# SketchyScene/SketchySceneColorization

Hardware: AMD Instinct MI355X
Metric: train images/sec (192x192, gen+disc fwd+bwd) (higher is better)
Workload: dtype fp32 (bf16x6 split on the bf16 MFMA, fp32 accumulate; filter gradients and few-channel layers on the exact-fp32 MFMA)

## Files before the change

include/sketchycolor_hip.h:

```cpp
#ifndef SKETCHYCOLOR_HIP_H
#define SKETCHYCOLOR_HIP_H

#include <stdint.h>

#ifdef __cplusplus
extern "C" {
#endif

#define SSC_ACT_NONE 0
#define SSC_ACT_RELU 1
#define SSC_ACT_LRELU 2
#define SSC_ACT_TANH 3
#define SSC_ACT_PRELU 5
#define SSC_ACT_MIU 4

typedef struct ssc_gview {
    const float* s0;
    const float* s1;
    const float* ab0;
    const float* ab1;
    int32_t C0, C1;
    int32_t H, W;
    int32_t act;
    int32_t act1;
// ... 46 lines not shown
    void* dst;
    int32_t taps, c0, c1, orient;
    int64_t first_thread;
} ssc_split_job;
int ssc_filter_split_geom(int taps, int c0, int c1, int orient, int* kc, int* nbp, int64_t* bytes, int64_t* threads);
int ssc_filter_split(const float* w, int taps, int c0, int c1, int orient, void* dst, void* stream);
int ssc_bf16_prepare(void);
int ssc_filter_split_batch(const ssc_split_job* jobs_dev, int njobs, int64_t total_threads, void* stream);

int ssc_sk_configure(int timeout_ms, int test_withhold);

typedef struct ssc_wgrad_desc {
    ssc_gview g;
    ssc_gview d;
    float* out;
    int32_t NB, PH, PW;
    int32_t TH, TW, in_stride, ioff_y, ioff_x;
    int32_t Cg_real;
    int32_t Nn;
    int32_t ldc;
    int32_t accumulate;
    int32_t exact;
    int32_t _pad;
} ssc_wgrad_desc;

int ssc_version(void);
int ssc_build_hash(char* buf, int len);
int ssc_device_info(int* cu_count, int* wave_size, char* arch, int arch_len);

int ssc_conv_forward(const ssc_conv_desc* d, float* ws, int64_t ws_bytes, void* stream);
int ssc_conv_wgrad(const ssc_wgrad_desc* d, float* ws, int64_t ws_bytes, void* stream);
int ssc_conv_wgrad128_supported(const ssc_wgrad_desc* d);
int ssc_conv_wgrad128(const ssc_wgrad_desc* d, float* ws, int64_t ws_bytes, void* stream);
int ssc_conv_wgn16_supported(const ssc_wgrad_desc* d);
int ssc_conv_forward_bn(const ssc_conv_desc* d, float* ws, int64_t ws_bytes, const float* scale, const float* offset,
                        float eps, float* ab, float* stats, void* stream);
int ssc_head1_forward_supported(const ssc_conv_desc* d);
int ssc_head1_forward(const ssc_conv_desc* d, float* ws, int64_t ws_bytes, void* stream);
int ssc_head1_dgrad_supported(const ssc_conv_desc* d);
int ssc_head1_dgrad(const ssc_conv_desc* d, void* stream);
int ssc_head1_wgrad_supported(const ssc_wgrad_desc* d);
int ssc_head1_wgrad(const ssc_wgrad_desc* d, float* ws, int64_t ws_bytes, void* stream);
int ssc_head1_dgrad_bn_backward(const ssc_conv_desc* d, const float* x, const float* ab, const float* stats, int act,
                                const float* rowb, float rowb_scale, float* dx, float* dscale, float* doffset, float* ws,
                                int64_t ws_bytes, void* stream);
int ssc_bn_bwd_finalize(const float* partial, int nblk, int C, int64_t M, float* coef, float* dscale, float* doffset,
                        void* stream);
int ssc_conv_narrow_supported(const ssc_conv_desc* d);
int ssc_conv_narrow_forward(const ssc_conv_desc* d, void* stream);
int ssc_conv_pw1x1_supported(const ssc_conv_desc* d);
int ssc_conv_c3x3_supported(const ssc_conv_desc* d);
int ssc_conv_s2n16_supported(const ssc_conv_desc* d);
int ssc_conv_tr4n16_supported(const ssc_conv_desc* d);
int ssc_conv_fewchan7_supported(const ssc_conv_desc* d);
int ssc_conv_tr4_tiny_supported(const ssc_conv_desc* d);
int ssc_conv_fewchan_supported(const ssc_conv_desc* d);
int ssc_conv_forward_kernel_name(const ssc_conv_desc* d, char* buf, int len);
int ssc_conv_wgrad_kernel_name(const ssc_wgrad_desc* d, char* buf, int len);
int ssc_conv_forward_plan(const ssc_conv_desc* d, int64_t ws_bytes, int* out5);
int ssc_conv_wgrad_plan(const ssc_wgrad_desc* d, int64_t ws_bytes, int* out4);
int ssc_conv_wgrad128_plan(const ssc_wgrad_desc* d, int64_t ws_bytes, int* out7);
int ssc_conv_bf_plan(const ssc_conv_desc* d, int64_t ws_bytes, int* out10);

int ssc_nchw_to_nhwc(const float* src, float* dst, int N, int C, int HW, int ldc, int coff, void* stream);
int ssc_nhwc_to_nchw(const float* src, float* dst, int N, int C, int HW, int ldc, int coff, void* stream);
int ssc_sketch_preprocess_u8(const uint8_t* src, int N, int H, int W, int thicken, float* dst, void* stream);
int ssc_image_postprocess_u8(const float* src, int ldc, int coff, int64_t M, uint8_t* dst, void* stream);
int ssc_bg_stage_u8(const uint8_t* fg, const uint8_t* bg, const int32_t* labels, int64_t M, float* inputs, float* targets,
                    float* xd_real, float* count, void* workspace, int64_t workspace_bytes, void* stream);
int ssc_bg_stage_cached_u8(const uint8_t* fg_cache, int64_t S_fg, const uint8_t* bg_cache, int64_t S_bg, const uint8_t* seg_cache,
                           int64_t S_seg, const int32_t* slot, const uint8_t* recolor, int64_t N, int64_t P, float* inputs,
                           float* targets, float* xd_real, int32_t* labels, float* count, void* workspace,
                           int64_t workspace_bytes, void* stream);
int ssc_bg_finish_u8(const float* img, int ldc, const uint8_t* fg, const uint8_t* mask, int64_t M, uint8_t* out,
                     void* stream);
int ssc_image_metrics_u8(const uint8_t* a, const uint8_t* b, const uint8_t* mask, int N, int H, int W, const double* win11,
                         double* out, void* ws, int64_t ws_bytes, void* stream);
int ssc_image_metrics_f32(const float* a, int lda, int coff_a, const float* b, int ldb, int coff_b, int b_planar, int N, int H,
                          int W, const double* win11, double* out, void* ws, int64_t ws_bytes, void* stream);
int ssc_image_metrics_bg_f32(const float* img, int ldc, const uint8_t* fg, const uint8_t* target, const uint8_t* mask, int N, int H,
                             int W, const double* win11, double* out, void* ws, int64_t ws_bytes, void* stream);
int ssc_seg_confusion(const float* logits, int ld, int K, const int32_t* labels, int64_t N, int64_t P, int64_t* out, void* ws,
                      int64_t ws_bytes, void* stream);
int ssc_bg_scene_crop_u8(const uint8_t* prev, const uint8_t* inner, int64_t M, uint8_t* fg_out, void* stream);
int ssc_bg_scene_compose_u8(const float* img, int ldc, const uint8_t* fg, const uint8_t* inner, const uint8_t* grass,
                            const uint8_t* sketch, int H, int W, uint8_t* out, uint8_t* fg_marked, int overlay_only,
                            void* stream);
int ssc_bg_sky_gradient_u8(const uint8_t* color, const uint8_t* inner, int H, int W, int search_from, int search_height,
                           uint8_t* out, int32_t* status, void* workspace, int64_t workspace_bytes, void* stream);
int ssc_fg_scene_mask_u8(const uint8_t* small_mask, int bh, int bw, uint8_t* out, void* stream);
int ssc_road_parallel_u8(const uint8_t* sketch, int S, int parallel_width, int32_t* out, void* stream);
int ssc_fg_scene_paste_u8(uint8_t* result, const uint8_t* inner, int H, int W, const uint8_t* inst, int y1, int x1, int bh, int bw,
                          int value, void* stream);
int ssc_resample_u8(const uint8_t* src, int H, int W, int C, int chan, const int32_t* bnd_h, const int32_t* k_h, int ks_h,
                    int new_w, const int32_t* bnd_v, const int32_t* k_v, int ks_v, int new_h, uint8_t* tmp, uint8_t* dst,
                    int OH, int OW, int OC, int top, int left, int fill, void* stream);
int ssc_decode_paired_u8(const uint8_t* img, const uint8_t* sk, const float* sk_f32, int N, int R, int size,
                         const float* noise, float* img_out, float* sk_out, float* mnmx, void* stream);
int ssc_decode_minmax_u8(const uint8_t* img, int N, int R, int size, float* mnmx, void* stream);
int ssc_decode_paired_cached_u8(const uint8_t* img_cache, const uint8_t* sk_cache, const float* skf_cache,
                                const float* mnmx_cache, int64_t S, const int32_t* idx, int N, int R, int size,
                                const float* noise, float* img_out, float* sk_out, void* stream);
int ssc_distance_map_u8(const uint8_t* sk, int N, int R, float* out, int32_t* ws, int64_t ws_bytes, void* stream);
uint32_t ssc_crc32c(const uint8_t* data, int64_t n);
int ssc_fill(float* dst, float value, int64_t n, void* stream);
int ssc_timestamp(uint64_t* dst, void* stream);
// ... 206 lines not shown
```

sketchyscenecolorization_amd/build.py:

```python
import os
import subprocess
import sys

HERE = os.path.dirname(os.path.abspath(__file__))
ROOT = os.path.dirname(HERE)
CSRC = os.path.join(HERE, 'csrc')
LIB_DIR = os.path.join(HERE, 'lib')
LIB_PATH = os.path.join(LIB_DIR, 'libsketchycolor_hip.so')
EXTRA_FLAGS = {'igemm.hip': ['-Xclang', '-target-feature', '-Xclang', '-load-store-opt']} if os.environ.get('SSC_NO_LSOPT') == '1' else {}
NO_PACKED_FP32 = {'narrow.hip': []}
VGPR_FORM = ['-mllvm', '-amdgpu-mfma-vgpr-form=1']
LAST_BUILD = None
SOURCES = ['igemm.hip', 'igemm_bf16.hip', 'wgrad128.hip', 'wgrad128_bf16.hip', 'wgn16.hip', 'narrow.hip', 'head1.hip', 'fewchan.hip', 'fewchan7.hip', 'pw1x1.hip', 'c3x3.hip', 's2n16.hip', 'tr4tiny.hip', 'tr4n16.hip', 'elementwise.hip', 'text_lstm.hip', 'losses_optim.hip', 'mru_ops.hip', 'bg_io.hip', 'bg_scene.hip', 'fg_scene.hip', 'metrics.hip', 'matching.hip', 'match_eval.hip', 'match_train.hip', 'match_val.hip', 'match_backbone_train.hip', 'match_attn.hip', 'match_segnet.hip']


def _hipcc():
    for c in (os.environ.get('HIPCC'), '/opt/rocm/bin/hipcc', 'hipcc'):
        if c and (os.path.isabs(c) and os.path.exists(c) or not os.path.isabs(c)):
            return c
    return 'hipcc'


HASH_MARKER = b'SSC_CSRC_HASH='


def tree_hash(csrc=None, header=None):
    import hashlib
    csrc = csrc or CSRC
    header = header or os.path.join(ROOT, 'include', 'sketchycolor_hip.h')
    h = hashlib.sha256()
    for fp in [os.path.join(csrc, f) for f in sorted(os.listdir(csrc))] + [header]:
        if fp.endswith(('.hip', '.h')):
            with open(fp, 'rb') as fh:
                h.update(os.path.basename(fp).encode() + b'\0' + fh.read())
    return h.hexdigest()[:16]


def library_hash(path=None):
    path = path or LIB_PATH
    if not os.path.exists(path):
        return None
    with open(path, 'rb') as fh:
        blob = fh.read()
    i = blob.find(HASH_MARKER)
    if i < 0:
        return None
    return blob[i + len(HASH_MARKER):i + len(HASH_MARKER) + 16].decode('ascii', 'replace')


def is_stale():
    return library_hash() != tree_hash()


def build_library(force=False, verbose=True):
    global LAST_BUILD
    if not force and not is_stale():
        LAST_BUILD = 'reused'
        return LIB_PATH
    LAST_BUILD = 'rebuilt'
    os.makedirs(LIB_DIR, exist_ok=True)
    th = tree_hash()
    import hashlib
    objs = []
    procs = []
    hdrs = b''
    for hp in sorted(os.path.join(CSRC, f) for f in os.listdir(CSRC) if f.endswith('.h')) + [os.path.join(ROOT, 'include', 'sketchycolor_hip.h')]:
# ... 36 lines not shown
```

sketchyscenecolorization_amd/csrc/igemm.hip:

```cpp
#include <hip/hip_runtime.h>
#include <stdint.h>
#include <stdio.h>
#include <stdlib.h>
#include "sketchycolor_hip.h"
#include "igemm_util.h"
#include "igemm_epilogue.h"
#include "host_util.h"

extern "C" int ssc_conv_wgrad128_supported(const ssc_wgrad_desc* dp);
extern "C" int ssc_conv_wgrad128(const ssc_wgrad_desc* dp, float* ws, int64_t ws_bytes, void* stream);
int ssc_conv_wgrad128_bf_selected(const ssc_wgrad_desc* dp);
extern "C" int ssc_conv_wgn16_supported(const ssc_wgrad_desc* dp);
int ssc_conv_wgn16(const ssc_wgrad_desc* dp, float* ws, int64_t ws_bytes, void* stream);
int ssc_conv_wgn16_fits(const ssc_wgrad_desc* dp, int64_t ws_bytes);
int ssc_conv_narrow_forward_ws(const ssc_conv_desc* dp, float* ws, int64_t ws_bytes, void* stream, int* csplit_out);
int ssc_conv_fewchan_forward(const ssc_conv_desc* dp, int num_cu, void* stream);
extern "C" int ssc_conv_pw1x1_supported(const ssc_conv_desc* dp);
int ssc_conv_pw1x1_walkers(const ssc_conv_desc* dp);
int ssc_conv_pw1x1_forward(const ssc_conv_desc* dp, float* stat, void* stream);
extern "C" int ssc_conv_tr4n16_supported(const ssc_conv_desc* dp);
int ssc_conv_tr4n16_rows(const ssc_conv_desc* dp);
int ssc_conv_tr4n16_forward(const ssc_conv_desc* dp, float* stat, void* stream);
extern "C" int ssc_conv_fewchan7_supported(const ssc_conv_desc* dp);
int ssc_conv_fewchan7_walkers(const ssc_conv_desc* dp);
int ssc_conv_fewchan7_forward(const ssc_conv_desc* dp, float* stat, void* stream);
extern "C" int ssc_conv_tr4_tiny_supported(const ssc_conv_desc* dp);
int ssc_conv_tr4_tiny_blocks(const ssc_conv_desc* dp);
int ssc_conv_tr4_tiny_forward(const ssc_conv_desc* dp, float* stat, void* stream);
extern "C" int ssc_conv_s2n16_supported(const ssc_conv_desc* dp);
int ssc_conv_s2n16_walkers(const ssc_conv_desc* dp);
int ssc_conv_s2n16_forward(const ssc_conv_desc* dp, float* stat, void* stream);
extern "C" int ssc_conv_c3x3_supported(const ssc_conv_desc* dp);
int ssc_conv_c3x3_walkers(const ssc_conv_desc* dp);
int ssc_conv_c3x3_forward(const ssc_conv_desc* dp, float* stat, void* stream);

bool ssc_bf_hk_enabled();
int ssc_launch_conv_bf(int cfg, bool plain, const ssc_conv_desc& d, int splitk, float* ws, hipStream_t st, long ts_full, int ts_s,
                       int64_t ws_bytes, int xcd);
int ssc_conv_bf_form(int cfg, bool plain, const ssc_conv_desc& d, int splitk, bool have_ws, long ts_full, int ts_s, int64_t ws_bytes,
                     int xcd, int* out10);
int ssc_sk_configure_bf(const unsigned* cfg4);

#define BK 32
__device__ unsigned g_sk_cfg[4] = {2000000000u, 0u, 0u, 0u};
#ifndef SSC_BDMA
#define SSC_BDMA 1
#endif
#ifndef SSC_ADMA
#define SSC_ADMA 0
#endif
#ifndef SSC_UT_SGB
#define SSC_UT_SGB 1
#endif

template <int WM, int WN, int SM, int SN, int BMODE, bool VECB>
__global__ __launch_bounds__(256) void conv_fwd_kernel(const ssc_conv_desc d, const Magics mg,
                                                        float* __restrict__ slab_base, long slab_stride,
                                                        int splitk) {
    constexpr int BM = WM * SM * 32;
    constexpr int BN = WN * SN * 32;
    constexpr int A_LD = BK + 1;
    constexpr int A_SZ = BM * A_LD;
    constexpr int B_LD = (BMODE == 0) ? BN : (BK + 1);
    constexpr int B_SZ = (BMODE == 0) ? BK * BN : BN * (BK + 1);
    constexpr int A_ROWS = BM / 32;
    constexpr int B_SLOTS = BN / 32;
    constexpr int B_RP = 1024 / BN;
    static_assert(WM * WN == 4, "4 waves per workgroup");

    extern __shared__ __attribute__((aligned(16))) float smem[];
    float* As = smem;
    float* Bs = smem + 2 * A_SZ;
    long* rowpix = reinterpret_cast<long*>(smem + 2 * A_SZ + 2 * B_SZ);

    const int tid = threadIdx.x;
// ... 1379 lines not shown
        const char* e = getenv("SSC_ARITH");
        off = (e != nullptr && (e[0] == 'f' || e[0] == 'F')) ? 1 : 0;
    }
    const bool km = d.x.C1 == 0 && (d.x.C0 & 3) == 0 && d.x.C0 > BK && (d.x.C0 % BK) != 0 && d.k_real >= 1 && d.k_real <= d.x.C0 &&
                    d.ws_kc == 2 * ((d.x.C0 + BK - 1) / BK) && (long)d.NB * d.x.H * d.x.W * d.x.C0 < 0x1fffffffL &&
                    (long)d.KH * d.KW * d.wC0 * d.wC1 < 0x1fffffffL;
    return !off && d.wsplit != nullptr && d.ws_kc > 0 && d.ws_nbp > 0 && (fwd_is_ut(d) || km) && (d.n_off & 31) == 0 && d.Nstore > 32 &&
           d.TH * d.TW <= 32;
}

static Plan plan_fwd(const ssc_conv_desc& d, int64_t ws_bytes, bool have_ws) {
    const long M = (long)d.NB * d.PH * d.PW;
    const int C = d.x.C0 + d.x.C1;
    long nkt = ((long)d.TH * d.TW * C + BK - 1) / BK;
    if (fwd_is_ut(d) || fwd_is_utg(d))
        nkt = (long)d.TH * d.TW * ((d.x.C0 + BK - 1) / BK + (d.x.C1 + BK - 1) / BK);
    else if (d.bmode == 0 && fwd_is_rowtap(d))
        nkt = d.TH;
    const bool allowed[5] = {d.Nstore > 64, d.Nstore > 64, d.Nstore > 32, d.Nstore <= 32, d.Nstore > 32};
    const bool can_ts = d.sk_flags != nullptr && tail_split_mode() != 0 &&
                        (fwd_is_ut(d) || fwd_is_utg(d) || (d.bmode == 0 && fwd_is_rowtap(d)));
    if (fwd_is_bf(d)) {
        const bool allowed_bf[5] = {d.Nstore > 64, d.Nstore > 64, true, false, true};
        TileCfg cfgs[5];
        for (int i = 0; i < 5; ++i) cfgs[i] = BF_CFGS[i];
        if (ssc_bf_hk_enabled()) {
            const long t128 = ((M + 127) / 128) * ((d.Nstore + 127) / 128) * d.nphase;
            if ((double)t128 < plan_const("SSC_PLAN_BF_HK_MIN", 0.5) * 2.0 * num_cu()) {
                return plan_launch(cfgs, 5, allowed_bf, M, d.Nstore, d.nphase, nkt, (long)d.NB * d.OH * d.OW * d.ldc, ws_bytes,
                                   have_ws, can_ts, plan_const("SSC_PLAN_BF_SCALE", 0.45));
            }
            cfgs[0].res = 2;
            cfgs[0].penalty = plan_const("SSC_PLAN_BF_HK", 0.78);
            if (!fwd_is_ut(d)) cfgs[0].penalty *= (double)((d.x.C0 + 15) / 16) / (double)(2 * ((d.x.C0 + 31) / 32));
        }
        return plan_launch(cfgs, 5, allowed_bf, M, d.Nstore, d.nphase, nkt, (long)d.NB * d.OH * d.OW * d.ldc, ws_bytes,
                           have_ws, can_ts, plan_const("SSC_PLAN_BF_SCALE", 0.45));
    }
    return plan_launch(FWD_CFGS, 5, allowed, M, d.Nstore, d.nphase, nkt, (long)d.NB * d.OH * d.OW * d.ldc, ws_bytes,
                       have_ws, can_ts);
}

static void copy_name(const char* src, char* dst, int len) {
    int i = 0;
    for (; i < len - 1 && src[i]; ++i) dst[i] = src[i];
    if (len > 0) dst[i] = 0;
}

extern "C" int ssc_conv_forward_kernel_name(const ssc_conv_desc* dp, char* buf, int len) {
    if (ssc_head1_forward_supported(dp) || ssc_head1_dgrad_supported(dp)) {
        copy_name(ssc_head1_dgrad_supported(dp) ? "head1_dgrad" : "head1_fwd", buf, len);
        return 0;
    }
    if (ssc_conv_narrow_supported(dp)) {
        copy_name(dp->nphase == 4 ? "narrow_fwd<transposed>" : "narrow_fwd<conv>", buf, len);
        return 0;
    }
    if (ssc_conv_fewchan_supported(dp)) {
        copy_name(dp->x.C0 == 8 ? "conv_fewchan<8>" : "conv_fewchan<4>", buf, len);
        return 0;
    }
    if (ssc_conv_pw1x1_supported(dp)) {
        copy_name("conv_pw1x1", buf, len);
        return 0;
    }
    if (ssc_conv_c3x3_supported(dp)) {
        copy_name(dp->bmode ? "conv_c3x3<NK>" : "conv_c3x3<KN>", buf, len);
        return 0;
    }
    if (ssc_conv_s2n16_supported(dp)) {
        copy_name("conv_s2n16", buf, len);
        return 0;
    }
    if (ssc_conv_tr4_tiny_supported(dp)) {
        copy_name("deconv_tr4_tiny", buf, len);
        return 0;
    }
    if (ssc_conv_fewchan7_supported(dp)) {
        copy_name("conv_fewchan7", buf, len);
        return 0;
    }
    if (ssc_conv_tr4n16_supported(dp)) {
        copy_name("deconv_tr4n16", buf, len);
        return 0;
    }
    static const char* names[2][5] = {
        {"conv_fwd<128x128,KN>", "conv_fwd<64x128,KN>", "conv_fwd<128x64,KN>", "conv_fwd<128x32,KN>", "conv_fwd<64x64,KN>"},
        {"conv_fwd<128x128,NK>", "conv_fwd<64x128,NK>", "conv_fwd<128x64,NK>", "conv_fwd<128x32,NK>", "conv_fwd<64x64,NK>"}};
    const Plan p = plan_fwd(*dp, (int64_t)1 << 40, true);
    if (fwd_is_bf(*dp)) {
        static const char* bfn[5] = {"conv_bf16x6<128x128>", "conv_bf16x6<64x128>", "conv_bf16x6<128x64>", "conv_bf16x6<128x32>",
                                     "conv_bf16x6<64x64>"};
        copy_name(bfn[p.cfg < 0 ? 0 : p.cfg], buf, len);
        return 0;
    }
    copy_name(names[dp->bmode ? 1 : 0][p.cfg < 0 ? 0 : p.cfg], buf, len);
    return 0;
}

extern "C" int ssc_bn_stats(const float* x, int64_t M, int C, int ldx, const float* scale, const float* offset, float eps,
                            float* ab, float* stats, float* ws, int64_t ws_bytes, void* stream);
extern "C" int ssc_bn_finalize(const float* partial, int nblk, int C, int64_t M, const float* scale, const float* offset,
                               float eps, float* ab, float* stats, void* stream);

extern "C" int ssc_conv_forward_bn(const ssc_conv_desc* dp, float* ws, int64_t ws_bytes, const float* scale,
                                   const float* offset, float eps, float* ab, float* stats, void* stream) {
// ... 192 lines not shown
        const char* e = ssc_dev_getenv("SSC_FUSE_BNBWD");
        off = (e != nullptr && e[0] == '0') ? 1 : 0;
    }
    const int C1 = d.Nstore - C0;
    if (!off && ws != nullptr && s0 != nullptr && s1 != nullptr && s0->x && s1->x && s0->ab && s1->ab && s0->stats && s1->stats &&
        s0->partial && s1->partial && C0 > 0 && C1 > 0 && (C0 % 128) == 0 && (C1 & 3) == 0 &&
        !ssc_conv_narrow_supported(dp) && !ssc_conv_fewchan_supported(dp) && d.epi == 0 && !d.accumulate &&
        d.bias == nullptr && d.Nstore == d.ldc && d.Nn == d.Nstore && ((s0->ldx | s1->ldx) & 3) == 0 &&
        ((reinterpret_cast<unsigned long>(d.out) | reinterpret_cast<unsigned long>(s0->x) |
          reinterpret_cast<unsigned long>(s1->x)) & 15) == 0 &&
        (fwd_is_ut(d) || fwd_is_utg(d))) {
        const Plan p = plan_fwd(d, ws_bytes, true);
        if (p.cfg >= 0 && p.splitk == 1 && FWD_CFGS[p.cfg].BN <= 128) {
            const long mt = (M + FWD_CFGS[p.cfg].BM - 1) / FWD_CFGS[p.cfg].BM;
            if ((int64_t)mt * d.nphase * 2 * C0 * 4 <= s0->partial_bytes && (int64_t)mt * d.nphase * 2 * C1 * 4 <= s1->partial_bytes) {
                d.stat_partial = s0->partial;
                d.sb_x = s0->x; d.sb_ldx = s0->ldx; d.sb_ab = s0->ab; d.sb_stats = s0->stats; d.sb_act = s0->act;
                d.stat_partial2 = s1->partial; d.sb2_col0 = C0;
                d.sb2_x = s1->x; d.sb2_ldx = s1->ldx; d.sb2_ab = s1->ab; d.sb2_stats = s1->stats; d.sb2_act = s1->act;
                *nrows = (int)(mt * d.nphase);
            }
        }
    }
    return ssc_conv_forward(&d, ws, ws_bytes, stream);
}

extern "C" int ssc_sk_configure(int timeout_ms, int test_withhold) {
    const unsigned long long ticks = (unsigned long long)(timeout_ms > 0 ? timeout_ms : 20000) * 100000ull;
    const unsigned cfg[4] = {(unsigned)(ticks & 0xffffffffu), (unsigned)(ticks >> 32), test_withhold ? 1u : 0u, 0u};
    const int rc = ssc_sk_configure_bf(cfg);
    if (rc != 0) return rc;
    return (int)hipMemcpyToSymbol(HIP_SYMBOL(g_sk_cfg), cfg, sizeof(cfg), 0, hipMemcpyHostToDevice);
}

extern "C" int ssc_conv_forward_plan(const ssc_conv_desc* dp, int64_t ws_bytes, int* out5) {
    if (ssc_conv_narrow_supported(dp) || ssc_conv_fewchan_supported(dp)) {
        out5[0] = -1; out5[1] = 1; out5[2] = 0; out5[3] = 1; out5[4] = 0;
        return 0;
    }
    const Plan p = plan_fwd(*dp, ws_bytes, true);
    out5[0] = p.cfg; out5[1] = p.splitk; out5[2] = (int)p.ts_full; out5[3] = p.ts_s; out5[4] = (int)(p.cost / 1000.0);
    return 0;
}

static int fwd_desc_error(const ssc_conv_desc& d) {
    if ((d.x.C0 & 3) || (d.x.C1 & 3) || d.Nstore < d.Nn || d.Nstore > d.ldc) return -1;
    if (d.nphase != 1 && d.nphase != 4) return -2;
    if (d.nphase == 4 && (d.TH != 2 || d.TW != 2 || d.KH != 4 || d.KW != 4 || d.kstep != -2 || d.out_stride != 2 ||
                          d.in_stride != 1))
        return -3;
    return 0;
}
enum { FWD_TILED = 0, FWD_HEAD1, FWD_HEAD1_DGRAD, FWD_NARROW, FWD_FEWCHAN, FWD_PW1X1, FWD_C3X3, FWD_S2N16, FWD_TR4_TINY, FWD_FEWCHAN7,
       FWD_TR4N16 };
static int fwd_early_kernel(const ssc_conv_desc* dp, bool have_ws, int64_t ws_bytes) {
    const ssc_conv_desc& d = *dp;
    if (have_ws && ssc_head1_forward_supported(dp) && (int64_t)d.NB * d.x.H * d.x.W * 16 * 4 <= ws_bytes) return FWD_HEAD1;
    if (ssc_head1_dgrad_supported(dp)) return FWD_HEAD1_DGRAD;
    if (ssc_conv_narrow_supported(dp)) return FWD_NARROW;
    if (ssc_conv_fewchan_supported(dp)) return FWD_FEWCHAN;
    if (ssc_conv_pw1x1_supported(dp)) return FWD_PW1X1;
    if (ssc_conv_c3x3_supported(dp)) return FWD_C3X3;
    if (ssc_conv_s2n16_supported(dp)) return FWD_S2N16;
    if (ssc_conv_tr4_tiny_supported(dp)) return FWD_TR4_TINY;
    if (ssc_conv_fewchan7_supported(dp)) return FWD_FEWCHAN7;
    if (ssc_conv_tr4n16_supported(dp)) return FWD_TR4N16;
    return FWD_TILED;
}
static bool fwd_bf_plain(const ssc_conv_desc& d) {
    const bool plain0 = d.x.ab0 == nullptr && d.x.act == SSC_ACT_NONE;
    const bool plain1 = d.x.C1 == 0 || (d.x.ab1 == nullptr && (d.x.act1 >= 0 ? d.x.act1 : d.x.act) == SSC_ACT_NONE);
    return plain0 && plain1;
}

extern "C" int ssc_conv_bf_plan(const ssc_conv_desc* dp, int64_t ws_bytes, int* out10) {
    const ssc_conv_desc& d = *dp;
    const bool have_ws = ws_bytes > 0;
    const int err = fwd_desc_error(d);
    if (err != 0) return err;
    if (fwd_early_kernel(dp, have_ws, ws_bytes) != FWD_TILED || !fwd_is_bf(d)) return -10;
    const Plan p = plan_fwd(d, ws_bytes, have_ws);
    if (p.cfg < 0) return -4;
    return ssc_conv_bf_form(p.cfg, fwd_bf_plain(d), d, p.splitk, have_ws, p.ts_full, p.ts_s, ws_bytes, xcd_order(), out10);
}

extern "C" int ssc_conv_forward(const ssc_conv_desc* dp, float* ws, int64_t ws_bytes, void* stream) {
    const ssc_conv_desc& d = *dp;
    hipStream_t st = (hipStream_t)stream;
    const int err = fwd_desc_error(d);
    if (err != 0) return err;
    switch (fwd_early_kernel(dp, ws != nullptr, ws_bytes)) {
        case FWD_HEAD1: return ssc_head1_forward(dp, ws, ws_bytes, stream);
        case FWD_HEAD1_DGRAD: return ssc_head1_dgrad(dp, stream);
        case FWD_NARROW: {
            int csplit = 1;
            const int rc = ssc_conv_narrow_forward_ws(dp, ws, ws_bytes, stream, &csplit);
            if (rc != 0 || csplit == 1) return rc;
            const long out_count = (long)d.NB * d.OH * d.OW * d.ldc;
            hipLaunchKernelGGL(slab_reduce_kernel, dim3((unsigned)((out_count + 255) / 256)), dim3(256), 0, st, ws, out_count,
                               csplit, d.out, out_count, d.ldc, d.Nn, d.Nstore, d.bias, d.epi, d.accumulate);
            return (int)hipGetLastError();
        }
        case FWD_FEWCHAN: return ssc_conv_fewchan_forward(dp, num_cu(), stream);
        case FWD_PW1X1: return ssc_conv_pw1x1_forward(dp, d.stat_partial, stream);
        case FWD_C3X3: return ssc_conv_c3x3_forward(dp, d.stat_partial, stream);
        case FWD_S2N16: return ssc_conv_s2n16_forward(dp, d.stat_partial, stream);
        case FWD_TR4_TINY: return ssc_conv_tr4_tiny_forward(dp, d.stat_partial, stream);
        case FWD_FEWCHAN7: return ssc_conv_fewchan7_forward(dp, d.stat_partial, stream);
        case FWD_TR4N16: return ssc_conv_tr4n16_forward(dp, d.stat_partial, stream);
        default: break;
    }
    const Plan p = plan_fwd(d, ws_bytes, ws != nullptr);
    if (p.cfg < 0) return -4;
    if (fwd_is_bf(d)) return ssc_launch_conv_bf(p.cfg, fwd_bf_plain(d), d, p.splitk, ws, st, p.ts_full, p.ts_s, ws_bytes, xcd_order());
    g_launch_res = FWD_CFGS[p.cfg].res;
    g_launch_ws_bytes = ws_bytes;
    g_launch_ts_full = p.ts_full;
    g_launch_ts_s = p.ts_s;
    if (d.bmode == 0) {
        switch (p.cfg) {
            case 0: return launch_fwd<2, 2, 2, 2, 0>(d, p.splitk, ws, st);
            case 1: return launch_fwd<2, 2, 1, 2, 0>(d, p.splitk, ws, st);
            case 2: return launch_fwd<2, 2, 2, 1, 0>(d, p.splitk, ws, st);
            case 4: return launch_fwd<2, 2, 1, 1, 0>(d, p.splitk, ws, st);
            default: return launch_fwd<4, 1, 1, 1, 0>(d, p.splitk, ws, st);
        }
    } else {
        switch (p.cfg) {
            case 0: return launch_fwd<2, 2, 2, 2, 1>(d, p.splitk, ws, st);
            case 1: return launch_fwd<2, 2, 1, 2, 1>(d, p.splitk, ws, st);
            case 2: return launch_fwd<2, 2, 2, 1, 1>(d, p.splitk, ws, st);
            case 4: return launch_fwd<2, 2, 1, 1, 1>(d, p.splitk, ws, st);
            default: return launch_fwd<4, 1, 1, 1, 1>(d, p.splitk, ws, st);
        }
    }
}

static bool gview_plain(const ssc_gview& g) {
    return g.ab0 == nullptr && g.act == SSC_ACT_NONE &&
           (g.C1 == 0 || (g.ab1 == nullptr && (g.act1 >= 0 ? g.act1 : g.act) == SSC_ACT_NONE));
}

template <int WM, int WN, int SM, int SN, bool GPLAIN, bool DPLAIN, bool DDMA>
static int launch_wgrad_v(const ssc_wgrad_desc& d, int splitk, float* ws, hipStream_t st) {
    constexpr int BM = WM * SM * 32, BN = WN * SN * 32;
    constexpr size_t lds = 2 * (BK * BM + BK * BN) * sizeof(float) + 2 * BK * sizeof(int4);
// ... 156 lines not shown
```

sketchyscenecolorization_amd/hip.py:

```python
import ctypes as C
import os

import torch

_HERE = os.path.dirname(os.path.abspath(__file__))
LIB_PATH = os.environ.get('SSC_LIB_PATH') or os.path.join(_HERE, 'lib', 'libsketchycolor_hip.so')

ACT_PRELU = 5
ACT_NONE, ACT_RELU, ACT_LRELU, ACT_TANH, ACT_MIU = 0, 1, 2, 3, 4


class GView(C.Structure):
    _fields_ = [('s0', C.c_void_p), ('s1', C.c_void_p), ('ab0', C.c_void_p), ('ab1', C.c_void_p),
                ('C0', C.c_int32), ('C1', C.c_int32), ('H', C.c_int32), ('W', C.c_int32),
                ('act', C.c_int32), ('act1', C.c_int32)]


class ConvDesc(C.Structure):
    _fields_ = [('x', GView), ('w', C.c_void_p), ('bias', C.c_void_p), ('out', C.c_void_p),
                ('NB', C.c_int32), ('PH', C.c_int32), ('PW', C.c_int32),
                ('TH', C.c_int32), ('TW', C.c_int32), ('in_stride', C.c_int32),
                ('ioff_y', C.c_int32), ('ioff_x', C.c_int32), ('nphase', C.c_int32),
                ('ky0', C.c_int32), ('kx0', C.c_int32), ('kstep', C.c_int32),
                ('KH', C.c_int32), ('KW', C.c_int32), ('wC0', C.c_int32), ('wC1', C.c_int32),
# ... 75 lines not shown
    if have != want:
        msg = ('%s was built from kernel sources %s, the tree is %s: rebuild (python -m sketchyscenecolorization_amd.build)'
               % (LIB_PATH, have, want))
        if os.environ.get('SSC_ALLOW_STALE_LIB') == '1':
            import warnings
            warnings.warn(msg)
        else:
            raise RuntimeError(msg)
    return have


_P, _I, _L, _F = C.c_void_p, C.c_int, C.c_int64, C.c_float

SIGNATURES = {
    'ssc_version': [],
    'ssc_build_hash': [C.c_char_p, _I],
    'ssc_device_info': [C.POINTER(C.c_int), C.POINTER(C.c_int), C.c_char_p, _I],
    'ssc_conv_forward': [C.POINTER(ConvDesc), _P, _L, _P],
    'ssc_filter_split_geom': [_I, _I, _I, _I, C.POINTER(C.c_int), C.POINTER(C.c_int), C.POINTER(C.c_int64), C.POINTER(C.c_int64)],
    'ssc_filter_split': [_P, _I, _I, _I, _I, _P, _P],
    'ssc_filter_split_batch': [_P, _I, _L, _P],
    'ssc_bf16_prepare': [],
    'ssc_conv_wgrad': [C.POINTER(WgradDesc), _P, _L, _P],
    'ssc_conv_wgrad128_supported': [C.POINTER(WgradDesc)],
    'ssc_conv_wgn16_supported': [C.POINTER(WgradDesc)],
    'ssc_conv_wgrad128': [C.POINTER(WgradDesc), _P, _L, _P],
    'ssc_conv_forward_bn': [C.POINTER(ConvDesc), _P, _L, _P, _P, _F, _P, _P, _P],
    'ssc_bn_finalize': [_P, _I, _I, _L, _P, _P, _F, _P, _P, _P],
    'ssc_conv_forward_bnbwd': [C.POINTER(ConvDesc), _P, _L, _P, _I, _P, _P, _I, _P, _L, C.POINTER(C.c_int), _P],
    'ssc_conv_forward_minmax': [C.POINTER(ConvDesc), _P, _L, _P, _P],
    'ssc_minmax_finalize': [_P, _I, _I, _I, _P, _P],
    'ssc_conv_forward_bnbwd2': [C.POINTER(ConvDesc), _P, _L, C.POINTER(BnBwdSite), C.POINTER(BnBwdSite), _I,
                                C.POINTER(C.c_int), _P],
    'ssc_bn_act_backward_pre': [_P, _L, _I, _I, _P, _P, _P, _I, _I, _P, _I, _I, _I, _P, _I, _P, _P, _P, _I, _P, _F, _I, _P,
                                _L, _P],
    'ssc_head1_forward_supported': [C.POINTER(ConvDesc)],
    'ssc_head1_forward': [C.POINTER(ConvDesc), _P, _L, _P],
    'ssc_head1_dgrad_supported': [C.POINTER(ConvDesc)],
    'ssc_head1_dgrad': [C.POINTER(ConvDesc), _P],
    'ssc_head1_wgrad_supported': [C.POINTER(WgradDesc)],
    'ssc_head1_wgrad': [C.POINTER(WgradDesc), _P, _L, _P],
    'ssc_head1_dgrad_bn_backward': [C.POINTER(ConvDesc), _P, _P, _P, _I, _P, _F, _P, _P, _P, _P, _L, _P],
    'ssc_bn_bwd_finalize': [_P, _I, _I, _L, _P, _P, _P, _P],
    'ssc_block_out_backward': [_P, _P, _L, _I, _I, _P, _P, _P, _P, _P, _P, _P, _P, _P, _P, _P, _P, _P, _P, _P, _L, _P],
    'ssc_bn_bwd_sums': [C.POINTER(BnApplyJob), _P, _I, _P, _P, _P, _P, _L, _P],
    'ssc_bn_bwd_apply': [C.POINTER(BnApplyJob), _P],
    'ssc_conv_narrow_supported': [C.POINTER(ConvDesc)],
    'ssc_conv_narrow_forward': [C.POINTER(ConvDesc), _P],
    'ssc_conv_fewchan_supported': [C.POINTER(ConvDesc)],
    'ssc_conv_pw1x1_supported': [C.POINTER(ConvDesc)],
    'ssc_conv_c3x3_supported': [C.POINTER(ConvDesc)],
    'ssc_conv_s2n16_supported': [C.POINTER(ConvDesc)],
    'ssc_conv_tr4n16_supported': [C.POINTER(ConvDesc)],
    'ssc_conv_fewchan7_supported': [C.POINTER(ConvDesc)],
    'ssc_conv_tr4_tiny_supported': [C.POINTER(ConvDesc)],
    'ssc_conv_forward_kernel_name': [C.POINTER(ConvDesc), C.c_char_p, _I],
    'ssc_conv_wgrad_kernel_name': [C.POINTER(WgradDesc), C.c_char_p, _I],
    'ssc_conv_forward_plan': [C.POINTER(ConvDesc), _L, C.POINTER(C.c_int)],
    'ssc_conv_wgrad_plan': [C.POINTER(WgradDesc), _L, C.POINTER(C.c_int)],
    'ssc_conv_wgrad128_plan': [C.POINTER(WgradDesc), _L, C.POINTER(C.c_int)],
    'ssc_conv_bf_plan': [C.POINTER(ConvDesc), _L, C.POINTER(C.c_int)],
    'ssc_sk_configure': [_I, _I],
    'ssc_nchw_to_nhwc': [_P, _P, _I, _I, _I, _I, _I, _P],
    'ssc_nhwc_to_nchw': [_P, _P, _I, _I, _I, _I, _I, _P],
    'ssc_sketch_preprocess_u8': [_P, _I, _I, _I, _I, _P, _P],
    'ssc_image_postprocess_u8': [_P, _I, _I, _L, _P, _P],
    'ssc_bg_stage_u8': [_P, _P, _P, _L, _P, _P, _P, _P, _P, _L, _P],
    'ssc_bg_stage_cached_u8': [_P, _L, _P, _L, _P, _L, _P, _P, _L, _L, _P, _P, _P, _P, _P, _P, _L, _P],
    'ssc_bg_finish_u8': [_P, _I, _P, _P, _L, _P, _P],
    'ssc_bg_scene_crop_u8': [_P, _P, _L, _P, _P],
    'ssc_bg_scene_compose_u8': [_P, _I, _P, _P, _P, _P, _I, _I, _P, _P, _I, _P],
    'ssc_bg_sky_gradient_u8': [_P, _P, _I, _I, _I, _I, _P, _P, _P, _L, _P],
    'ssc_fg_scene_mask_u8': [_P, _I, _I, _P, _P],
    'ssc_road_parallel_u8': [_P, _I, _I, _P, _P],
    'ssc_fg_scene_paste_u8': [_P, _P, _I, _I, _P, _I, _I, _I, _I, _I, _P],
    'ssc_image_metrics_u8': [_P, _P, _P, _I, _I, _I, _P, _P, _P, _L, _P],
    'ssc_image_metrics_f32': [_P, _I, _I, _P, _I, _I, _I, _I, _I, _I, _P, _P, _P, _L, _P],
    'ssc_image_metrics_bg_f32': [_P, _I, _P, _P, _P, _I, _I, _I, _P, _P, _P, _L, _P],
    'ssc_seg_confusion': [_P, _I, _I, _P, _L, _L, _P, _P, _L, _P],
    'ssc_resample_u8': [_P, _I, _I, _I, _I, _P, _P, _I, _I, _P, _P, _I, _I, _P, _P, _I, _I, _I, _I, _I, _I, _P],
    'ssc_decode_paired_u8': [_P, _P, _P, _I, _I, _I, _P, _P, _P, _P, _P],
    'ssc_decode_minmax_u8': [_P, _I, _I, _I, _P, _P],
    'ssc_decode_paired_cached_u8': [_P, _P, _P, _P, _L, _P, _I, _I, _I, _P, _P, _P, _P],
    'ssc_distance_map_u8': [_P, _I, _I, _P, _P, _L, _P],
    'ssc_fill': [_P, _F, _L, _P],
    'ssc_timestamp': [_P, _P],
    'ssc_affine_act': [_P, _I, _P, _I, _I, _P, _I, _L, _I, _P],
    'ssc_residual_merge': [_P, _P, _P, _P, _I, _P, _L, _I, _P],
    'ssc_bn_stats': [_P, _L, _I, _I, _P, _P, _F, _P, _P, _P, _L, _P],
    'ssc_bn_act_backward': [_P, _L, _I, _I, _P, _P, _P, _P, _I, _I, _P, _I, _I, _I, _P, _I, _P, _P, _P, _L, _P],
    'ssc_embedding_gather': [_P, _P, _I, _I, _P, _P],
    'ssc_embedding_scatter_add': [_P, _I, _P, _I, _I, _P, _P],
    'ssc_row_l2norm_fwd': [_P, _I, _P, _L, _I, _P, _P, _P],
    'ssc_row_l2norm_bwd': [_P, _P, _P, _L, _I, _P, _I, _P],
    'ssc_lstm_pointwise_fwd': [_P, _P, _P, _I, _P, _I, _P, _P, _L, _I, _P, _P, _P, _P],
    'ssc_lstm_step_fwd': [_P, _P, _I, _P, _P, _I, _P, _I, _P, _L, _I, _I, _P, _P, _P, _P],
    'ssc_lstm_step_fwd_bf': [_P, _P, _P, _I, _P, _P, _I, _P, _I, _P, _L, _I, _P, _P, _P, _P, _P],
    'ssc_lstm_hsplit': [_P, _L, _I, _P, _P],
    'ssc_lstm_pointwise_bwd': [_P, _P, _P, _P, _P, _P, _I, _L, _I, _P, _P, _P, _P, _P],
    'ssc_squash_fwd': [_P, _L, _P, _P],
    'ssc_squash_bwd': [_P, _P, _P, _L, _P, _P],
    'ssc_group_rowsum': [_P, _I, _L, _I, _I, _P, _I, _P],
    'ssc_act_mean_hw': [_P, _P, _I, _I, _I, _I, _P, _P],
    'ssc_add_row_bcast': [_P, _P, _F, _I, _I, _I, _P],
    'ssc_miu_permute_fwd': [_P, _I, _I, _I, _P, _P],
    'ssc_miu_permute_bwd': [_P, _P, _I, _I, _I, _P, _P],
# ... 1571 lines not shown
```

Measured before the change: 2420.

## Add fp32-MFMA transposed 4x4 stride-2 conv kernel for 1-3 output channels

Adds a dedicated kernel for transposed 4x4 stride-2 convolutions with up to three output channels, such as the RGB output head. Each 16x16 input tile, with affine and activation applied on load, is staged in shared memory. All 16 taps times 3 outputs are computed as one small GEMM on the exact-fp32 MFMA, and the four phase outputs are then gathered from shared memory. It takes priority over the narrow kernel path. The cost is a persistent-walker schedule and a specialised code path with tight applicability checks.

```diff
diff --git a/include/sketchycolor_hip.h b/include/sketchycolor_hip.h
--- a/include/sketchycolor_hip.h
+++ b/include/sketchycolor_hip.h
@@ -122,6 +122,8 @@
 int ssc_conv_c3x3_supported(const ssc_conv_desc* d);
 int ssc_conv_s2n16_supported(const ssc_conv_desc* d);
 int ssc_conv_tr4n16_supported(const ssc_conv_desc* d);
+int ssc_conv_tr4n3_supported(const ssc_conv_desc* d);
+int ssc_conv_tr4n3_forward(const ssc_conv_desc* d, void* stream);
 int ssc_conv_fewchan7_supported(const ssc_conv_desc* d);
 int ssc_conv_tr4_tiny_supported(const ssc_conv_desc* d);
 int ssc_conv_fewchan_supported(const ssc_conv_desc* d);
diff --git a/sketchyscenecolorization_amd/build.py b/sketchyscenecolorization_amd/build.py
--- a/sketchyscenecolorization_amd/build.py
+++ b/sketchyscenecolorization_amd/build.py
@@ -11,7 +11,7 @@
 NO_PACKED_FP32 = {'narrow.hip': []}
 VGPR_FORM = ['-mllvm', '-amdgpu-mfma-vgpr-form=1']
 LAST_BUILD = None
-SOURCES = ['igemm.hip', 'igemm_bf16.hip', 'wgrad128.hip', 'wgrad128_bf16.hip', 'wgn16.hip', 'narrow.hip', 'head1.hip', 'fewchan.hip', 'fewchan7.hip', 'pw1x1.hip', 'c3x3.hip', 's2n16.hip', 'tr4tiny.hip', 'tr4n16.hip', 'elementwise.hip', 'text_lstm.hip', 'losses_optim.hip', 'mru_ops.hip', 'bg_io.hip', 'bg_scene.hip', 'fg_scene.hip', 'metrics.hip', 'matching.hip', 'match_eval.hip', 'match_train.hip', 'match_val.hip', 'match_backbone_train.hip', 'match_attn.hip', 'match_segnet.hip']
+SOURCES = ['igemm.hip', 'igemm_bf16.hip', 'wgrad128.hip', 'wgrad128_bf16.hip', 'wgn16.hip', 'narrow.hip', 'head1.hip', 'fewchan.hip', 'fewchan7.hip', 'pw1x1.hip', 'c3x3.hip', 's2n16.hip', 'tr4tiny.hip', 'tr4n16.hip', 'tr4n3.hip', 'elementwise.hip', 'text_lstm.hip', 'losses_optim.hip', 'mru_ops.hip', 'bg_io.hip', 'bg_scene.hip', 'fg_scene.hip', 'metrics.hip', 'matching.hip', 'match_eval.hip', 'match_train.hip', 'match_val.hip', 'match_backbone_train.hip', 'match_attn.hip', 'match_segnet.hip']
 
 
 def _hipcc():
diff --git a/sketchyscenecolorization_amd/csrc/igemm.hip b/sketchyscenecolorization_amd/csrc/igemm.hip
--- a/sketchyscenecolorization_amd/csrc/igemm.hip
+++ b/sketchyscenecolorization_amd/csrc/igemm.hip
@@ -21,6 +21,8 @@
 extern "C" int ssc_conv_tr4n16_supported(const ssc_conv_desc* dp);
 int ssc_conv_tr4n16_rows(const ssc_conv_desc* dp);
 int ssc_conv_tr4n16_forward(const ssc_conv_desc* dp, float* stat, void* stream);
+extern "C" int ssc_conv_tr4n3_supported(const ssc_conv_desc* dp);
+extern "C" int ssc_conv_tr4n3_forward(const ssc_conv_desc* dp, void* stream);
 extern "C" int ssc_conv_fewchan7_supported(const ssc_conv_desc* dp);
 int ssc_conv_fewchan7_walkers(const ssc_conv_desc* dp);
 int ssc_conv_fewchan7_forward(const ssc_conv_desc* dp, float* stat, void* stream);
@@ -1506,6 +1508,10 @@
         copy_name(ssc_head1_dgrad_supported(dp) ? "head1_dgrad" : "head1_fwd", buf, len);
         return 0;
     }
+    if (ssc_conv_tr4n3_supported(dp)) {
+        copy_name("tr4n3<fp32 mfma>", buf, len);
+        return 0;
+    }
     if (ssc_conv_narrow_supported(dp)) {
         copy_name(dp->nphase == 4 ? "narrow_fwd<transposed>" : "narrow_fwd<conv>", buf, len);
         return 0;
@@ -1804,11 +1810,12 @@
     return 0;
 }
 enum { FWD_TILED = 0, FWD_HEAD1, FWD_HEAD1_DGRAD, FWD_NARROW, FWD_FEWCHAN, FWD_PW1X1, FWD_C3X3, FWD_S2N16, FWD_TR4_TINY, FWD_FEWCHAN7,
-       FWD_TR4N16 };
+       FWD_TR4N16, FWD_TR4N3 };
 static int fwd_early_kernel(const ssc_conv_desc* dp, bool have_ws, int64_t ws_bytes) {
     const ssc_conv_desc& d = *dp;
     if (have_ws && ssc_head1_forward_supported(dp) && (int64_t)d.NB * d.x.H * d.x.W * 16 * 4 <= ws_bytes) return FWD_HEAD1;
     if (ssc_head1_dgrad_supported(dp)) return FWD_HEAD1_DGRAD;
+    if (ssc_conv_tr4n3_supported(dp)) return FWD_TR4N3;
     if (ssc_conv_narrow_supported(dp)) return FWD_NARROW;
     if (ssc_conv_fewchan_supported(dp)) return FWD_FEWCHAN;
     if (ssc_conv_pw1x1_supported(dp)) return FWD_PW1X1;
@@ -1844,6 +1851,7 @@
     switch (fwd_early_kernel(dp, ws != nullptr, ws_bytes)) {
         case FWD_HEAD1: return ssc_head1_forward(dp, ws, ws_bytes, stream);
         case FWD_HEAD1_DGRAD: return ssc_head1_dgrad(dp, stream);
+        case FWD_TR4N3: return ssc_conv_tr4n3_forward(dp, stream);
         case FWD_NARROW: {
             int csplit = 1;
             const int rc = ssc_conv_narrow_forward_ws(dp, ws, ws_bytes, stream, &csplit);
diff --git a/sketchyscenecolorization_amd/csrc/tr4n3.hip b/sketchyscenecolorization_amd/csrc/tr4n3.hip
--- /dev/null
+++ b/sketchyscenecolorization_amd/csrc/tr4n3.hip
@@ -0,0 +1,255 @@
+#include <hip/hip_runtime.h>
+#include <stdint.h>
+#include <stdlib.h>
+#include "sketchycolor_hip.h"
+#include "host_util.h"
+
+typedef float f32x4 __attribute__((ext_vector_type(4)));
+
+#define N3_PT 16
+#define N3_IT (N3_PT - 2)
+#define N3_CH 32
+#define N3_PST 36
+#define N3_STG (N3_PT * N3_PT * N3_PST)
+#define N3_TST 52
+#define N3_LDS (2 * N3_STG * 4 + 2 * 128 * 4)
+
+__device__ __forceinline__ float n3_act(float v, float slope, unsigned keep) {
+    return fmaxf(v, __uint_as_float(__float_as_uint(slope * v) & keep));
+}
+
+template <int NCHUNK>
+__global__ __launch_bounds__(256) __attribute__((amdgpu_waves_per_eu(2))) void tr4n3_kernel(const ssc_conv_desc d, int tiles, int tiles_x,
+                                                                                            int tiles_y) {
+    extern __shared__ __attribute__((aligned(16))) float smem[];
+    const int tid = threadIdx.x, lane = tid & 63, wave = tid >> 6;
+    const int l15 = lane & 15, kq = lane >> 4;
+    const int H = d.x.H, W = d.x.W;
+
+    constexpr int C = N3_CH * NCHUNK;
+
+    float* const abl = smem + 2 * N3_STG;
+    if (tid < C) {
+        const bool first = tid < d.x.C0;
+        const float* abp = first ? d.x.ab0 : d.x.ab1;
+        const int cs = first ? d.x.C0 : d.x.C1;
+        const int cc = first ? tid : tid - d.x.C0;
+        abl[tid] = abp != nullptr ? abp[cc] : 1.f;
+        abl[C + tid] = abp != nullptr ? abp[cs + cc] : 0.f;
+    }
+
+    const int c4s = (tid & 7) * 4;
+    const int pcol = (tid >> 3) & 15;
+    const int prow = __builtin_amdgcn_readfirstlane(tid >> 7);
+    int t_n = 0, t_iy0 = 0, t_ix = 0;
+    auto set_tile = [&](int tile) {
+        const int txi = tile % tiles_x;
+        const int r = tile / tiles_x;
+        const int tyi = r % tiles_y;
+        t_n = r / tiles_y;
+        t_iy0 = N3_IT * tyi - 1 + prow;
+        t_ix = N3_IT * txi - 1 + pcol;
+    };
+    float4 rv[8];
+    auto load_chunk = [&](int cb) {
+        const bool first = cb < d.x.C0;
+        const float* src = first ? d.x.s0 : d.x.s1;
+        const int cs = first ? d.x.C0 : d.x.C1;
+        const int cc = first ? cb : cb - d.x.C0;
+        const int voff = min(max(t_ix, 0), W - 1) * cs + c4s;
+#pragma unroll
+        for (int q = 0; q < 8; ++q) {
+            const int iy = min(max(t_iy0 + 2 * q, 0), H - 1);
+            const float* rowp = src + ((long)(t_n * H + iy) * W) * cs + cc;
+            rv[q] = *reinterpret_cast<const float4*>(rowp + voff);
+        }
+    };
+    auto store_chunk = [&](float* stage, int cb) {
+        const int act = (cb >= d.x.C0 && d.x.act1 >= 0) ? d.x.act1 : d.x.act;
+        const float4 ra = *reinterpret_cast<const float4*>(abl + cb + c4s);
+        const float4 rb = *reinterpret_cast<const float4*>(abl + C + cb + c4s);
+        const bool colok = (unsigned)t_ix < (unsigned)W;
+        const float slope = act == SSC_ACT_LRELU ? 0.2f : 1.f;
+        const unsigned keep = act == SSC_ACT_RELU ? 0u : 0xffffffffu;
+#pragma unroll
+        for (int q = 0; q < 8; ++q) {
+            const int pos = (tid >> 3) + 32 * q;
+            float4 v = rv[q];
+            v.x = n3_act(fmaf(ra.x, v.x, rb.x), slope, keep); v.y = n3_act(fmaf(ra.y, v.y, rb.y), slope, keep);
+            v.z = n3_act(fmaf(ra.z, v.z, rb.z), slope, keep); v.w = n3_act(fmaf(ra.w, v.w, rb.w), slope, keep);
+            if (!(colok & ((unsigned)(t_iy0 + 2 * q) < (unsigned)H))) v = make_float4(0.f, 0.f, 0.f, 0.f);
+            *reinterpret_cast<float4*>(stage + pos * N3_PST + c4s) = v;
+        }
+    };
+
+    float bv[3];
+#pragma unroll
+    for (int n = 0; n < 3; ++n) bv[n] = (d.bias != nullptr && n < d.Nn) ? d.bias[n] : 0.f;
+
+    const int G = gridDim.x;
+    int tile = blockIdx.x;
+    if (tile >= tiles) return;
+    set_tile(tile);
+    load_chunk(0);
+
+    float bfr[3][8 * NCHUNK];
+    {
+        const long ks = (d.bmode == 0) ? (long)d.wC1 : 1L, ns = (d.bmode == 0) ? 1L : (long)d.wC1;
+        const float* wn0 = d.w + d.n_off * ns;
+        const long ts = (long)d.wC0 * d.wC1;
+#pragma unroll
+        for (int i = 0; i < 48 * C / 256; ++i) {
+            const int e = tid + 256 * i;
+            const int col = e / C, k = e - col * C;
+            const int tap = col / 3, n = col - 3 * tap;
+            const bool v = n < d.Nn;
+            const float wv = wn0[v ? tap * ts + n * ns + k * ks : 0];
+            smem[col * (C + 4) + k] = v ? wv : 0.f;
+        }
+        __syncthreads();
+#pragma unroll
+        for (int b = 0; b < 3; ++b)
+#pragma unroll
+            for (int s = 0; s < 8 * NCHUNK; ++s) bfr[b][s] = smem[(16 * b + l15) * (C + 4) + 4 * s + kq];
+        __syncthreads();
+    }
+
+    int buf = 0;
+    const int a_off = (4 * wave * N3_PT + l15) * N3_PST + kq;
+    for (; tile < tiles; tile += G) {
+        f32x4 acc[4][3];
+#pragma unroll
+        for (int g = 0; g < 4; ++g)
+#pragma unroll
+            for (int b = 0; b < 3; ++b) acc[g][b] = (f32x4){0.f, 0.f, 0.f, 0.f};
+#pragma unroll
+        for (int ch = 0; ch < NCHUNK; ++ch) {
+            float* stage = smem + buf * N3_STG;
+            store_chunk(stage, ch * N3_CH);
+            __syncthreads();
+            if (ch + 1 < NCHUNK) {
+                load_chunk((ch + 1) * N3_CH);
+            } else if (tile + G < tiles) {
+                set_tile(tile + G);
+                load_chunk(0);
+            }
+            const float* A0 = stage + a_off;
+#pragma unroll
+            for (int s = 0; s < 8; ++s) {
+#pragma unroll
+                for (int g = 0; g < 4; ++g) {
+                    const float a = A0[g * N3_PT * N3_PST + 4 * s];
+#pragma unroll
+                    for (int b = 0; b < 3; ++b) acc[g][b] = __builtin_amdgcn_mfma_f32_16x16x4f32(a, bfr[b][8 * ch + s], acc[g][b], 0, 0, 0);
+                }
+            }
+            buf ^= 1;
+        }
+        __syncthreads();
+#pragma unroll
+        for (int g = 0; g < 4; ++g)
+#pragma unroll
+            for (int b = 0; b < 3; ++b)
+#pragma unroll
+                for (int r = 0; r < 4; ++r) smem[(((4 * wave + g) * N3_PT) + 4 * kq + r) * N3_TST + 16 * b + l15] = acc[g][b][r];
+        __syncthreads();
+        {
+            const int txi = tile % tiles_x;
+            const int rr = tile / tiles_x;
+            const int tyi = rr % tiles_y, nimg = rr / tiles_y;
+#pragma unroll 1
+            for (int i = 0; i < (4 * N3_IT * N3_IT + 255) / 256; ++i) {
+                const int o = tid + 256 * i;
+                const int oy = o / (2 * N3_IT), ox = o - oy * (2 * N3_IT);
+                const int ly = oy >> 1, ry = oy & 1, lx = ox >> 1, rx = ox & 1;
+                const int py = N3_IT * tyi + ly, px = N3_IT * txi + lx;
+                if (o < 4 * N3_IT * N3_IT && py < d.PH && px < d.PW) {
+                    float sum[3] = {0.f, 0.f, 0.f};
+#pragma unroll
+                    for (int t = 0; t < 4; ++t) {
+                        const int ty = t >> 1, tx = t & 1;
+                        const int tap = (3 - ry - 2 * ty) * 4 + (3 - rx - 2 * tx);
+                        const float* tp = smem + ((ly + ry + ty) * N3_PT + lx + rx + tx) * N3_TST + 3 * tap;
+#pragma unroll
+                        for (int n = 0; n < 3; ++n) sum[n] += tp[n];
+                    }
+                    float* op = d.out + (((long)nimg * d.OH + 2 * py + ry) * d.OW + 2 * px + rx) * d.ldc;
+#pragma unroll
+                    for (int n = 0; n < 3; ++n) {
+                        if (n < d.Nn) {
+                            float v = sum[n];
+                            if (d.bias != nullptr) v += bv[n];
+                            if (d.epi == 1) v = tanhf(v);
+                            else if (d.epi == 2) v = fmaxf(v, 0.2f * v);
+                            if (d.accumulate) v += op[n];
+                            op[n] = v;
+                        } else if (n < d.Nstore) {
+                            op[n] = 0.f;
+                        }
+                    }
+                    if (d.Nstore > 3) op[3] = 0.f;
+                }
+            }
+        }
+        __syncthreads();
+    }
+}
+
+static bool n3_on() {
+    static int on = -1;
+    if (on < 0) {
+        const char* e = ssc_dev_getenv("SSC_TR4N3");
+        on = (e != nullptr && e[0] == '0') ? 0 : 1;
+    }
+    return on != 0;
+}
+
+extern "C" int ssc_conv_tr4n3_supported(const ssc_conv_desc* dp) {
+    const ssc_conv_desc& d = *dp;
+    if (!n3_on()) return 0;
+    if (d.nphase != 4 || d.TH != 2 || d.TW != 2 || d.KH != 4 || d.KW != 4 || d.kstep != -2 || d.out_stride != 2 || d.in_stride != 1)
+        return 0;
+    if (d.Nn < 1 || d.Nn > 3 || d.Nstore < d.Nn || d.Nstore > 4 || d.Nstore > d.ldc) return 0;
+    const int C = d.x.C0 + d.x.C1;
+    if (C < N3_CH || C > 4 * N3_CH || (C % N3_CH) != 0 || (d.x.C0 % N3_CH) != 0 || d.x.C0 < N3_CH || d.k_real != C) return 0;
+    if (d.bmode == 0 ? (d.wC0 < C || d.n_off + d.Nn > d.wC1) : (d.wC1 < C || d.n_off + d.Nn > d.wC0)) return 0;
+    if (d.n_off < 0 || d.OH != 2 * d.PH || d.OW != 2 * d.PW || d.x.H < 1 || d.x.W < 1 || d.PH < 1 || d.PW < 1 || d.NB < 1) return 0;
+    if ((reinterpret_cast<uintptr_t>(d.x.s0) & 15) != 0 || (d.x.C1 > 0 && (reinterpret_cast<uintptr_t>(d.x.s1) & 15) != 0)) return 0;
+    if ((d.x.ab0 != nullptr && (reinterpret_cast<uintptr_t>(d.x.ab0) & 15) != 0) ||
+        (d.x.C1 > 0 && d.x.ab1 != nullptr && (reinterpret_cast<uintptr_t>(d.x.ab1) & 15) != 0))
+        return 0;
+    if (d.stat_partial != nullptr || d.sb_x != nullptr || d.sb2_x != nullptr || d.stat_mode != 0) return 0;
+    const long ntile = (long)d.NB * ((d.PH + N3_IT - 1) / N3_IT) * ((d.PW + N3_IT - 1) / N3_IT);
+    if ((long)d.NB * d.x.H * d.x.W >= 0x7fffffffL || ntile >= 0x3fffffffL) return 0;
+    return 1;
+}
+
+static int n3_walkers(long tiles) {
+    const long g = 2L * ssc_num_cu();
+    if (tiles <= g) return (int)tiles;
+    const long rounds = (tiles + g - 1) / g;
+    return (int)((tiles + rounds - 1) / rounds);
+}
+
+extern "C" int ssc_conv_tr4n3_forward(const ssc_conv_desc* dp, void* stream) {
+    if (!ssc_conv_tr4n3_supported(dp)) return -1;
+    const ssc_conv_desc& d = *dp;
+    const int tiles_x = (d.PW + N3_IT - 1) / N3_IT, tiles_y = (d.PH + N3_IT - 1) / N3_IT;
+    const int tiles = d.NB * tiles_y * tiles_x;
+    const dim3 grid(n3_walkers(tiles));
+#define N3_LAUNCH(NC)                                                                                                      \
+    {                                                                                                                      \
+        static unsigned long long attr_done = 0;                                                                           \
+        const int arc = ssc_set_max_lds(reinterpret_cast<const void*>(&tr4n3_kernel<NC>), N3_LDS, &attr_done);             \
+        if (arc != 0) return arc;                                                                                          \
+        hipLaunchKernelGGL((tr4n3_kernel<NC>), grid, dim3(256), N3_LDS, (hipStream_t)stream, d, tiles, tiles_x, tiles_y);  \
+    }
+    switch ((d.x.C0 + d.x.C1) / N3_CH) {
+        case 1: N3_LAUNCH(1) break;
+        case 2: N3_LAUNCH(2) break;
+        case 3: N3_LAUNCH(3) break;
+        default: N3_LAUNCH(4) break;
+    }
+#undef N3_LAUNCH
+    return (int)hipGetLastError();
+}
diff --git a/sketchyscenecolorization_amd/hip.py b/sketchyscenecolorization_amd/hip.py
--- a/sketchyscenecolorization_amd/hip.py
+++ b/sketchyscenecolorization_amd/hip.py
@@ -151,6 +151,8 @@
     'ssc_conv_c3x3_supported': [C.POINTER(ConvDesc)],
     'ssc_conv_s2n16_supported': [C.POINTER(ConvDesc)],
     'ssc_conv_tr4n16_supported': [C.POINTER(ConvDesc)],
+    'ssc_conv_tr4n3_supported': [C.POINTER(ConvDesc)],
+    'ssc_conv_tr4n3_forward': [C.POINTER(ConvDesc), _P],
     'ssc_conv_fewchan7_supported': [C.POINTER(ConvDesc)],
     'ssc_conv_tr4_tiny_supported': [C.POINTER(ConvDesc)],
     'ssc_conv_forward_kernel_name': [C.POINTER(ConvDesc), C.c_char_p, _I],
```

After: 2416. No clear change (-0.2%).
